# gchochla/VAuLT

Measured on AMD Instinct MI355X. Metric: train samples/sec (img+text pairs) ViLT-B32+BERTweet, bs256, 1/2/4/8 MI355X, higher is better.
Workload: dtype bf16; 1 GPU; ViLT-B32 + bertweet fine-tune step (fwd+bwd+AdamW), per-GPU batch 256, 40 text tokens + 384x384 image (185-token fused sequence; resident as the patch-embedding operand `pixel_patches`, the input pipeline's output), all weights trained; global_batch=256, seq_len=185, parallelism=dp1

## Files before the change

vault_amd/csrc/norm.hip:

```cpp
#include <cstdlib>
#include <algorithm>
#include "common.h"
#include "../../include/vault_hip.h"

namespace {

struct RowMap {
  int rpg, gstride, goff;
  __device__ __forceinline__ size_t operator()(int r) const {
    if (rpg == 0) return (size_t)r;
    const int gq = r / rpg;
    return (size_t)gq * gstride + goff + (r - gq * rpg);
  }
};

template <int VPT>
__global__ __launch_bounds__(256) void ln_fwd_kernel(const float* __restrict__ x, RowMap xmap,
                                                     const float* __restrict__ gamma,
                                                     const float* __restrict__ beta, float eps, int rows, int H,
                                                     h16* __restrict__ y_bf16, float* __restrict__ y_f32, RowMap ymap,
                                                     const float* __restrict__ post_add,
                                                     float* __restrict__ mean, float* __restrict__ rstd,
                                                     uint32_t drop_thresh, uint32_t drop_seed, uint32_t drop_stream,
                                                     float drop_scale, h16* __restrict__ y_split3,
                                                     uint8_t* __restrict__ y_q, uint8_t* __restrict__ y_scale) {
  H16_SATURATE();
  const int lane = threadIdx.x & 63;
  const int row = blockIdx.x * 4 + (threadIdx.x >> 6);
  if (row >= rows) return;
  const float* xr = x + xmap(row) * H;
  f32x4 v[VPT];
  float s = 0.f;
#pragma unroll
  for (int j = 0; j < VPT; ++j) {
    v[j] = *reinterpret_cast<const f32x4*>(xr + (lane + 64 * j) * 4);
    s += v[j][0] + v[j][1] + v[j][2] + v[j][3];
  }
  const float mu = wave_sum(s) / (float)H;
  float q = 0.f;
#pragma unroll
  for (int j = 0; j < VPT; ++j)
#pragma unroll
    for (int e = 0; e < 4; ++e) {
      const float d = v[j][e] - mu;
      q += d * d;
    }
  const float var = wave_sum(q) / (float)H;
  const float rs = 1.0f / sqrtf(var + eps);
  if (lane == 0) {
    if (mean) mean[row] = mu;
    if (rstd) rstd[row] = rs;
  }
  const size_t orow = ymap(row);
#pragma unroll
  for (int j = 0; j < VPT; ++j) {
    const int c = (lane + 64 * j) * 4;
    const f32x4 gw = *reinterpret_cast<const f32x4*>(gamma + c);
    const f32x4 bw = *reinterpret_cast<const f32x4*>(beta + c);
    f32x4 o;
#pragma unroll
    for (int e = 0; e < 4; ++e) o[e] = (v[j][e] - mu) * rs * gw[e] + bw[e];
    if (drop_thresh != 0u) {
#pragma unroll
      for (int e = 0; e < 4; ++e)
        o[e] = dropout_keep(drop_seed, drop_stream, (uint32_t)(orow * H + c + e), drop_thresh) ? o[e] * drop_scale : 0.f;
    }
    if (post_add) {
      const f32x4 pa = *reinterpret_cast<const f32x4*>(post_add + c);
#pragma unroll
      for (int e = 0; e < 4; ++e) o[e] += pa[e];
    }
    if (y_f32) *reinterpret_cast<f32x4*>(y_f32 + orow * H + c) = o;
    if (y_bf16) {
      uint2 w = {pack_h16x2(o[0], o[1]), pack_h16x2(o[2], o[3])};
      *reinterpret_cast<uint2*>(y_bf16 + orow * H + c) = w;
    }
    if (y_q) {
      float b[4];
      float amax = 0.f;
#pragma unroll
      for (int e = 0; e < 4; ++e) { b[e] = (float)(h16)o[e]; amax = fmaxf(amax, fabsf(b[e])); }
      amax = fmaxf(amax, __shfl_xor(amax, 1, 64));
      amax = fmaxf(amax, __shfl_xor(amax, 2, 64));
      amax = fmaxf(amax, __shfl_xor(amax, 4, 64));
      int e8 = 0;
      if (amax > 0.f) {
        e8 = (int)((__builtin_bit_cast(uint32_t, amax) >> 23) & 0xff) - 8;
        e8 = e8 < 0 ? 0 : e8;
      }
      const float inv = __builtin_bit_cast(float, (uint32_t)(254 - e8) << 23);
#pragma unroll
      for (int e = 0; e < 4; ++e) b[e] = fminf(fmaxf(b[e] * inv, -448.f), 448.f);
      int w8 = 0;
      w8 = __builtin_amdgcn_cvt_pk_fp8_f32(b[0], b[1], w8, false);
      w8 = __builtin_amdgcn_cvt_pk_fp8_f32(b[2], b[3], w8, true);
      *reinterpret_cast<int*>(y_q + orow * H + c) = w8;
      if ((lane & 7) == 0) y_scale[orow * (H / 32) + (c >> 5)] = (uint8_t)e8;
    }
    if (y_split3) {
      h16 hi[4], lo[4];
#pragma unroll
      for (int e = 0; e < 4; ++e) split_bf16(o[e], hi[e], lo[e]);
      const uint2 wh = {pack_h16x2((float)hi[0], (float)hi[1]), pack_h16x2((float)hi[2], (float)hi[3])};
      const uint2 wl = {pack_h16x2((float)lo[0], (float)lo[1]), pack_h16x2((float)lo[2], (float)lo[3])};
      h16* d = y_split3 + orow * 3 * H + c;
      *reinterpret_cast<uint2*>(d) = wh;
      *reinterpret_cast<uint2*>(d + H) = wl;
      *reinterpret_cast<uint2*>(d + 2 * H) = wh;
    }
  }
}

template <int VPT, int WAVES>
__device__ __forceinline__ void ln_bwd_fold(const f32x4 (&ag)[VPT], const f32x4 (&ab)[VPT], const f32x4 (&ac)[VPT], float* red,
                                            float* dgamma, float* dbeta, float* dbias, int lane, int wave) {
  constexpr int NB = WAVES >= 8 ? 8 : 4;
  constexpr int HH = VPT * 256;
  if (dgamma == nullptr && dbias == nullptr) return;
  float* const dsts[3] = {dgamma, dbeta, dbias};
  for (int r = 0; r < WAVES / NB; ++r) {
    if ((wave / NB) == r) {
      float* rw = red + (wave % NB) * (3 * HH);
#pragma unroll
      for (int qn = 0; qn < 3; ++qn) {
        if (dsts[qn] == nullptr) continue;
#pragma unroll
        for (int j = 0; j < VPT; ++j) {
          const f32x4 v = qn == 0 ? ag[j] : (qn == 1 ? ab[j] : ac[j]);
          f32x4* q4 = reinterpret_cast<f32x4*>(rw + qn * HH + (lane + 64 * j) * 4);
          *q4 = (r == 0) ? v : (*q4 + v);
        }
      }
    }
    __syncthreads();
  }
  for (int c = threadIdx.x; c < 3 * HH; c += WAVES * 64) {
    const int qn = c / HH;
    float* dst = dsts[qn];
    if (dst == nullptr) continue;
    float t = 0.f;
#pragma unroll
    for (int b = 0; b < NB; ++b) t += red[b * (3 * HH) + c];
    atomicAdd(dst + (c - qn * HH), t);
  }
}

template <int VPT, int WAVES>
__global__ __launch_bounds__(WAVES * 64, 16 / WAVES) void ln_bwd_kernel(const h16* __restrict__ dy_bf16, const float* __restrict__ dy_f32,
                                                     RowMap dymap, const float* __restrict__ x, RowMap xmap,
                                                     const float* __restrict__ mean, const float* __restrict__ rstd,
                                                     const float* __restrict__ gamma, int rows, int H,
                                                     const float* __restrict__ dres, float* __restrict__ dx_f32,
                                                     h16* __restrict__ dx_bf16, RowMap dxmap, float* __restrict__ dgamma,
                                                     float* __restrict__ dbeta, float* __restrict__ dbias,
                                                     int rows_per_block, uint32_t drop_thresh, uint32_t drop_seed, uint32_t drop_stream,
                                                     float drop_scale, int drop_on_dy, const h16* __restrict__ dres_bf16) {
  H16_SATURATE();
  constexpr int NB = WAVES >= 8 ? 8 : 4;
  constexpr int HH = VPT * 256;
  extern __shared__ __attribute__((aligned(16))) float red[];
  const int lane = threadIdx.x & 63, wave = threadIdx.x >> 6;
  f32x4 gw[VPT], ag[VPT], ab[VPT], ac[VPT];
#pragma unroll
  for (int j = 0; j < VPT; ++j) {
    gw[j] = *reinterpret_cast<const f32x4*>(gamma + (lane + 64 * j) * 4);
    ag[j] = f32x4{0.f, 0.f, 0.f, 0.f};
    ab[j] = f32x4{0.f, 0.f, 0.f, 0.f};
    ac[j] = f32x4{0.f, 0.f, 0.f, 0.f};
  }
  const int r0 = blockIdx.x * rows_per_block;
  const int r1 = min(rows, r0 + rows_per_block);
  for (int row = r0 + wave; row < r1; row += WAVES) {
    const size_t xr = xmap(row) * H, dr = dymap(row) * H;
    const float mu = mean[row], rs = rstd[row];
    f32x4 xh[VPT], gy[VPT];
    float s1 = 0.f, s2 = 0.f;
#pragma unroll
    for (int j = 0; j < VPT; ++j) {
      const int c = (lane + 64 * j) * 4;
      const f32x4 xv = *reinterpret_cast<const f32x4*>(x + xr + c);
      f32x4 d = f32x4{0.f, 0.f, 0.f, 0.f};
      if (dy_f32) d = *reinterpret_cast<const f32x4*>(dy_f32 + dr + c);
      if (dy_bf16) {
        const uint2 w = *reinterpret_cast<const uint2*>(dy_bf16 + dr + c);
        const float2 a = unpack_h16x2(w.x), b = unpack_h16x2(w.y);
        d[0] += a.x; d[1] += a.y; d[2] += b.x; d[3] += b.y;
      }
      if (drop_on_dy && drop_thresh != 0u) {
#pragma unroll
        for (int e = 0; e < 4; ++e)
          d[e] = dropout_keep(drop_seed, drop_stream, (uint32_t)(dr + c + e), drop_thresh) ? d[e] * drop_scale : 0.f;
      }
#pragma unroll
      for (int e = 0; e < 4; ++e) {
        xh[j][e] = (xv[e] - mu) * rs;
        gy[j][e] = d[e] * gw[j][e];
        s1 += gy[j][e];
        s2 += gy[j][e] * xh[j][e];
        ag[j][e] += d[e] * xh[j][e];
        ab[j][e] += d[e];
      }
    }
    s1 = wave_sum(s1) / (float)H;
    s2 = wave_sum(s2) / (float)H;
    const size_t orow = dxmap(row) * H;
#pragma unroll
    for (int j = 0; j < VPT; ++j) {
      const int c = (lane + 64 * j) * 4;
      f32x4 o;
#pragma unroll
      for (int e = 0; e < 4; ++e) o[e] = rs * (gy[j][e] - s1 - xh[j][e] * s2);
      if (dres) {
        const f32x4 rv = *reinterpret_cast<const f32x4*>(dres + orow + c);
#pragma unroll
        for (int e = 0; e < 4; ++e) o[e] += rv[e];
      }
      if (dres_bf16) {
        const uint2 w = *reinterpret_cast<const uint2*>(dres_bf16 + orow + c);
        const float2 a = unpack_h16x2(w.x), b = unpack_h16x2(w.y);
        o[0] += a.x; o[1] += a.y; o[2] += b.x; o[3] += b.y;
      }
      if (dx_f32) *reinterpret_cast<f32x4*>(dx_f32 + orow + c) = o;
      if (dx_bf16) {
        if (drop_thresh != 0u && !drop_on_dy) {
#pragma unroll
          for (int e = 0; e < 4; ++e)
            o[e] = dropout_keep(drop_seed, drop_stream, (uint32_t)(orow + c + e), drop_thresh) ? o[e] * drop_scale : 0.f;
        }
        uint2 w = {pack_h16x2(o[0], o[1]), pack_h16x2(o[2], o[3])};
        *reinterpret_cast<uint2*>(dx_bf16 + orow + c) = w;
#pragma unroll
        for (int e = 0; e < 4; ++e) ac[j][e] += o[e];
      }
    }
  }
  ln_bwd_fold<VPT, WAVES>(ag, ab, ac, red, dgamma, dbeta, dbias, lane, wave);
}

template <int VPT>
__global__ __launch_bounds__(512, 1) void ln_bwd_stream_kernel(const h16* __restrict__ dy, const float* __restrict__ x,
                                                                const float* __restrict__ mean, const float* __restrict__ rstd,
                                                                const float* __restrict__ gamma, int rows, int H,
                                                                const h16* __restrict__ dres, h16* __restrict__ dx,
                                                                float* __restrict__ dgamma, float* __restrict__ dbeta,
                                                                float* __restrict__ dbias, int rows_per_block) {
  H16_SATURATE();
  constexpr int WAVES = 8;
  extern __shared__ __attribute__((aligned(16))) float red[];
  const int lane = threadIdx.x & 63, wave = threadIdx.x >> 6;
  f32x4 gw[VPT], ag[VPT], ab[VPT], ac[VPT];
#pragma unroll
  for (int j = 0; j < VPT; ++j) {
    gw[j] = *reinterpret_cast<const f32x4*>(gamma + (lane + 64 * j) * 4);
    ag[j] = f32x4{0.f, 0.f, 0.f, 0.f};
    ab[j] = f32x4{0.f, 0.f, 0.f, 0.f};
    ac[j] = f32x4{0.f, 0.f, 0.f, 0.f};
  }
  const int r0 = blockIdx.x * rows_per_block;
  const int r1 = min(rows, r0 + rows_per_block);
  struct RowRegs {
    f32x4 x[VPT];
    uint2 d[VPT], r[VPT];
    float mu, rs;
  };
  auto request = [&](RowRegs& q, int row) {
    const size_t o = (size_t)row * H;
#pragma unroll
    for (int j = 0; j < VPT; ++j) {
      const int c = (lane + 64 * j) * 4;
      q.x[j] = *reinterpret_cast<const f32x4*>(x + o + c);
      q.d[j] = *reinterpret_cast<const uint2*>(dy + o + c);
      q.r[j] = *reinterpret_cast<const uint2*>(dres + o + c);
    }
    q.mu = mean[row]; q.rs = rstd[row];
  };
  auto process = [&](const RowRegs& q, int row) {
    const float mu = q.mu, rs = q.rs;
    float s1 = 0.f, s2 = 0.f;
#pragma unroll
    for (int j = 0; j < VPT; ++j) {
      const float2 a = unpack_h16x2(q.d[j].x), b = unpack_h16x2(q.d[j].y);
      const float d[4] = {a.x, a.y, b.x, b.y};
#pragma unroll
      for (int e = 0; e < 4; ++e) {
        const float xh = (q.x[j][e] - mu) * rs;
        const float gy = d[e] * gw[j][e];
        s1 += gy;
        s2 += gy * xh;
        ag[j][e] += d[e] * xh;
        ab[j][e] += d[e];
      }
    }
    s1 = wave_sum(s1) / (float)H;
    s2 = wave_sum(s2) / (float)H;
    const size_t o = (size_t)row * H;
#pragma unroll
    for (int j = 0; j < VPT; ++j) {
      const int c = (lane + 64 * j) * 4;
      const float2 a = unpack_h16x2(q.d[j].x), b = unpack_h16x2(q.d[j].y);
      const float2 ra = unpack_h16x2(q.r[j].x), rb = unpack_h16x2(q.r[j].y);
      const float d[4] = {a.x, a.y, b.x, b.y};
      const float r[4] = {ra.x, ra.y, rb.x, rb.y};
      float out[4];
#pragma unroll
      for (int e = 0; e < 4; ++e) {
        const float xh = (q.x[j][e] - mu) * rs;
        out[e] = rs * (d[e] * gw[j][e] - s1 - xh * s2) + r[e];
        ac[j][e] += out[e];
      }
      uint2 w = {pack_h16x2(out[0], out[1]), pack_h16x2(out[2], out[3])};
      *reinterpret_cast<uint2*>(dx + o + c) = w;
    }
  };
  RowRegs qa, qb, qc;
  int row = r0 + wave;
  if (row < r1) request(qa, row);
  if (row + WAVES < r1) request(qb, row + WAVES);
  for (; row < r1; row += 3 * WAVES) {
    if (row + 2 * WAVES < r1) request(qc, row + 2 * WAVES);
    process(qa, row);
    if (row + WAVES >= r1) break;
    if (row + 3 * WAVES < r1) request(qa, row + 3 * WAVES);
    process(qb, row + WAVES);
    if (row + 2 * WAVES >= r1) break;
    if (row + 4 * WAVES < r1) request(qb, row + 4 * WAVES);
    process(qc, row + 2 * WAVES);
  }
  ln_bwd_fold<VPT, WAVES>(ag, ab, ac, red, dgamma, dbeta, dbias, lane, wave);
}

__global__ __launch_bounds__(1024) void colsum_kernel(const h16* __restrict__ in, int ld, int rows, int rows_per_block,
                                                      float* __restrict__ out, long long batch_in, long long batch_out) {
  __shared__ float red[16][256];
  in += (size_t)blockIdx.z * batch_in;
  out += (size_t)blockIdx.z * batch_out;
  const int lane = threadIdx.x & 63, wave = threadIdx.x >> 6;
  const int c0 = blockIdx.x * 256 + lane * 4;
  const int r0 = blockIdx.y * rows_per_block;
  const int r1 = min(rows, r0 + rows_per_block);
  float a0 = 0.f, a1 = 0.f, a2 = 0.f, a3 = 0.f;
  for (int r = r0 + wave; r < r1; r += 16) {
    const uint2 w = *reinterpret_cast<const uint2*>(in + (size_t)r * ld + c0);
    const float2 x = unpack_h16x2(w.x), y = unpack_h16x2(w.y);
    a0 += x.x; a1 += x.y; a2 += y.x; a3 += y.y;
  }
  red[wave][lane * 4] = a0; red[wave][lane * 4 + 1] = a1; red[wave][lane * 4 + 2] = a2; red[wave][lane * 4 + 3] = a3;
  __syncthreads();
  if (threadIdx.x < 256) {
    const int c = threadIdx.x;
    float t = 0.f;
#pragma unroll
    for (int w = 0; w < 16; ++w) t += red[w][c];
    atomicAdd(out + blockIdx.x * 256 + c, t);
  }
}

__global__ __launch_bounds__(1024) void colsum_hm_kernel(const h16* __restrict__ in, int rows, int hm_rows, int rows_per_block,
                                                         float* __restrict__ out, long long batch_in, long long batch_out) {
  __shared__ float red[128][65];
  const h16* base = in + (size_t)blockIdx.z * batch_in + (size_t)blockIdx.x * hm_rows * 64;
  const int t = threadIdx.x, r_in = t >> 3, c8 = (t & 7) * 8;
  const int r0 = blockIdx.y * rows_per_block, r1 = min(rows, r0 + rows_per_block);
  float a[8] = {0.f, 0.f, 0.f, 0.f, 0.f, 0.f, 0.f, 0.f};
  auto add = [&](const u32x4& w) {
#pragma unroll
    for (int k = 0; k < 4; ++k) {
      const float2 x = unpack_h16x2(w[k]);
      a[2 * k] += x.x; a[2 * k + 1] += x.y;
    }
  };
  int r = r0 + r_in;
  for (; r + 128 < r1; r += 256) {
    const u32x4 w0 = *reinterpret_cast<const u32x4*>(base + (size_t)r * 64 + c8);
    const u32x4 w1 = *reinterpret_cast<const u32x4*>(base + (size_t)(r + 128) * 64 + c8);
    add(w0); add(w1);
  }
  if (r < r1) add(*reinterpret_cast<const u32x4*>(base + (size_t)r * 64 + c8));
#pragma unroll
  for (int k = 0; k < 8; ++k) red[r_in][c8 + k] = a[k];
  __syncthreads();
  if (t < 64) {
    float s_ = 0.f;
#pragma unroll 8
    for (int q = 0; q < 128; ++q) s_ += red[q][t];
    atomicAdd(out + (size_t)blockIdx.z * batch_out + blockIdx.x * 64 + t, s_);
  }
}

}

extern "C" int vault_layernorm_fwd(const vault_ln_fwd_args* a, void* stream) {
  if (!a || a->H % 256 || (a->H > 1024 && a->H != 1536) || a->rows <= 0) return VAULT_EINVAL;
  hipStream_t st = reinterpret_cast<hipStream_t>(stream);
  const RowMap xm{a->x_rpg, a->x_gstride, a->x_goff}, ym{a->y_rpg, a->y_gstride, a->y_goff};
  dim3 grid((a->rows + 3) / 4), block(256);
#define LN_FWD(V)                                                                                          \
  hipLaunchKernelGGL(ln_fwd_kernel<V>, grid, block, 0, st, a->x, xm, a->gamma, a->beta, a->eps, a->rows,   \
                     a->H, reinterpret_cast<h16*>(a->y_bf16), a->y_f32, ym, a->post_add, a->mean, a->rstd, \
                     a->drop_thresh, a->drop_seed, a->drop_stream, a->drop_scale, reinterpret_cast<h16*>(a->y_split3), \
                     reinterpret_cast<uint8_t*>(a->y_q), reinterpret_cast<uint8_t*>(a->y_scale))
  switch (a->H / 256) {
    case 1: LN_FWD(1); break;
    case 2: LN_FWD(2); break;
    case 3: LN_FWD(3); break;
    case 4: LN_FWD(4); break;
    case 6: LN_FWD(6); break;
  }
#undef LN_FWD
  return (int)hipGetLastError();
}

extern "C" int vault_layernorm_bwd(const vault_ln_bwd_args* a, void* stream) {
  if (!a || a->H % 256 || (a->H > 1024 && a->H != 1536) || a->rows <= 0) return VAULT_EINVAL;
  hipStream_t st = reinterpret_cast<hipStream_t>(stream);
  const RowMap dym{a->dy_rpg, a->dy_gstride, a->dy_goff}, xm{a->x_rpg, a->x_gstride, a->x_goff},
      dxm{a->dx_rpg, a->dx_gstride, a->dx_goff};
  constexpr int waves = 16;
  const int maxb = 4096 / waves;
  int rpb = (a->rows + maxb - 1) / maxb;
  rpb = ((rpb + waves - 1) / waves) * waves;
  dim3 grid((a->rows + rpb - 1) / rpb), block(waves * 64);
  int lds_bytes = 0;
  const bool ident = a->dy_rpg == 0 && a->x_rpg == 0 && a->dx_rpg == 0;
  if (a->H == 768 && ident && a->dy_bf16 && !a->dy_f32 && !a->dres && a->dres_bf16 && !a->dx_f32 &&
      a->dx_bf16 && a->drop_thresh == 0 && a->dgamma && a->dbeta) {
    constexpr int LDS = 8 * 3 * 768 * 4;
    static bool done[64] = {};
    int dev = 0;
    if (hipGetDevice(&dev) != hipSuccess || dev < 0 || dev >= 64) return VAULT_EINVAL;
    if (!done[dev]) {
      if (hipFuncSetAttribute(reinterpret_cast<const void*>(&ln_bwd_stream_kernel<3>), hipFuncAttributeMaxDynamicSharedMemorySize,
                              LDS) != hipSuccess) return VAULT_EINVAL;
      done[dev] = true;
    }
    int rpb8 = (a->rows + 255) / 256;
    rpb8 = ((rpb8 + 7) / 8) * 8;
    hipLaunchKernelGGL((ln_bwd_stream_kernel<3>), dim3((a->rows + rpb8 - 1) / rpb8), dim3(512), LDS, st,
                       reinterpret_cast<const h16*>(a->dy_bf16), a->x, a->mean,
                       a->rstd, a->gamma, a->rows, a->H, reinterpret_cast<const h16*>(a->dres_bf16),
                       reinterpret_cast<h16*>(a->dx_bf16), a->dgamma, a->dbeta, a->dbias, rpb8);
    return (int)hipGetLastError();
  }
#define LN_BWD(V) LN_BWD_W(V, 16)
#define LN_BWD_W(V, W)                                                                                              \
  {                                                                                                                 \
  {                                                                                                                 \
    constexpr int LDS = (W >= 8 ? 8 : 4) * 3 * V * 256 * 4;                                                         \
    if (LDS > 64 * 1024) {                                                                                          \
      static bool done[64] = {};                                                                                    \
      int dev = 0;                                                                                                  \
      if (hipGetDevice(&dev) != hipSuccess || dev < 0 || dev >= 64) return VAULT_EINVAL;                            \
      if (!done[dev]) {                                                                                             \
        if (hipFuncSetAttribute(reinterpret_cast<const void*>(&ln_bwd_kernel<V, W>),                                \
                                hipFuncAttributeMaxDynamicSharedMemorySize, LDS) != hipSuccess) return VAULT_EINVAL; \
        done[dev] = true;                                                                                           \
      }                                                                                                             \
    }                                                                                                               \
    lds_bytes = LDS;                                                                                                \
  }                                                                                                                 \
  hipLaunchKernelGGL((ln_bwd_kernel<V, W>), grid, block, lds_bytes, st, reinterpret_cast<const h16*>(a->dy_bf16), a->dy_f32, \
                     dym, a->x, xm, a->mean, a->rstd, a->gamma, a->rows, a->H, a->dres, a->dx_f32,               \
                     reinterpret_cast<h16*>(a->dx_bf16), dxm, a->dgamma, a->dbeta, a->dbias, rpb, a->drop_thresh,          \
                     a->drop_seed, a->drop_stream, a->drop_scale, a->drop_on_dy, reinterpret_cast<const h16*>(a->dres_bf16)); \
  }
  switch (a->H / 256) {
    case 1: LN_BWD(1); break;
    case 2: LN_BWD(2); break;
    case 3: LN_BWD(3); break;
    case 4: LN_BWD(4); break;
    case 6: LN_BWD(6); break;
  }
#undef LN_BWD
#undef LN_BWD_W
  return (int)hipGetLastError();
}

__global__ __launch_bounds__(256) void colsum_partials_kernel(const float* __restrict__ part, int nparts, int n,
                                                              float* __restrict__ out, long long batch_in, long long batch_out) {
  const int c = blockIdx.x * 256 + threadIdx.x;
  if (c >= n) return;
  const int per = (nparts + (int)gridDim.z - 1) / (int)gridDim.z;
  const int r0 = blockIdx.z * per, r1 = min(nparts, r0 + per);
  const float* p = part + (size_t)blockIdx.y * batch_in + c;
  float a0 = 0.f, a1 = 0.f, a2 = 0.f, a3 = 0.f;
  int r = r0;
  for (; r + 3 < r1; r += 4) {
    a0 += p[(size_t)r * n]; a1 += p[(size_t)(r + 1) * n]; a2 += p[(size_t)(r + 2) * n]; a3 += p[(size_t)(r + 3) * n];
  }
  for (; r < r1; ++r) a0 += p[(size_t)r * n];
  if (r1 > r0) atomicAdd(out + (size_t)blockIdx.y * batch_out + c, (a0 + a1) + (a2 + a3));
}

extern "C" int vault_colsum_partials(const float* part, int nparts, int n, float* out, int batch, long long batch_in,
                                     long long batch_out, void* stream) {
  if (!part || !out || nparts <= 0 || n <= 0 || batch <= 0 || batch > 65535) return VAULT_EINVAL;
  const int slices = nparts >= 64 ? 16 : 1;
  hipLaunchKernelGGL(colsum_partials_kernel, dim3((n + 255) / 256, batch, slices), dim3(256), 0,
                     reinterpret_cast<hipStream_t>(stream), part, nparts, n, out, batch_in, batch_out);
  return (int)hipGetLastError();
}

extern "C" int vault_colsum_hm(const void* in_bf16, int rows, int hm_rows, int planes, float* out, int batch, long long batch_in,
                               long long batch_out, void* stream) {
  if (!in_bf16 || !out || rows <= 0 || hm_rows < rows || planes <= 0 || batch <= 0 || batch > 65535 || (batch_in & 3))
    return VAULT_EINVAL;
  const int row_blocks = std::max(4, 256 / (planes * batch));
  int rpb = (rows + row_blocks - 1) / row_blocks;
  rpb = ((rpb + 127) / 128) * 128;
  dim3 grid(planes, (rows + rpb - 1) / rpb, batch);
  hipLaunchKernelGGL(colsum_hm_kernel, grid, dim3(1024), 0, reinterpret_cast<hipStream_t>(stream),
                     reinterpret_cast<const h16*>(in_bf16), rows, hm_rows, rpb, out, batch_in, batch_out);
  return (int)hipGetLastError();
}

extern "C" int vault_colsum(const void* in_bf16, int ld, int rows, int N, float* out, void* stream) {
  if (!in_bf16 || !out || N % 256 || rows <= 0) return VAULT_EINVAL;
  const int row_blocks = 256;
  int rpb = (rows + row_blocks - 1) / row_blocks;
  rpb = ((rpb + 15) / 16) * 16;
  dim3 grid(N / 256, (rows + rpb - 1) / rpb);
  hipLaunchKernelGGL(colsum_kernel, grid, dim3(1024), 0, reinterpret_cast<hipStream_t>(stream),
                     reinterpret_cast<const h16*>(in_bf16), ld, rows, rpb, out, 0ll, 0ll);
  return (int)hipGetLastError();
}

extern "C" int vault_colsum_batched(const void* in_bf16, int ld, int rows, int N, float* out, int batch, long long batch_in,
                                    long long batch_out, void* stream) {
  if (!in_bf16 || !out || N % 256 || rows <= 0 || batch <= 0 || batch > 65535 || (batch_in & 3)) return VAULT_EINVAL;
  const int row_blocks = std::max(16, 256 / batch);
  int rpb = (rows + row_blocks - 1) / row_blocks;
  rpb = ((rpb + 15) / 16) * 16;
  dim3 grid(N / 256, (rows + rpb - 1) / rpb, batch);
  hipLaunchKernelGGL(colsum_kernel, grid, dim3(1024), 0, reinterpret_cast<hipStream_t>(stream),
                     reinterpret_cast<const h16*>(in_bf16), ld, rows, rpb, out, batch_in, batch_out);
  return (int)hipGetLastError();
}
```

vault_amd/csrc/optim.hip:

```cpp
#include "common.h"
#include "../../include/vault_hip.h"

namespace {

__global__ __launch_bounds__(256) void adamw_kernel(float* __restrict__ p, float* __restrict__ g, float* __restrict__ m,
                                                    float* __restrict__ v, h16* __restrict__ pb, long long n4,
                                                    float step_size, float lr_wd, float b1, float b2, float eps,
                                                    float gscale, int zero_grad, const uint8_t* __restrict__ zmask) {
  H16_SATURATE();
  for (long long i = blockIdx.x * 256ll + threadIdx.x; i < n4; i += (long long)gridDim.x * 256ll) {
    f32x4 pv = reinterpret_cast<f32x4*>(p)[i];
    f32x4 gv = reinterpret_cast<f32x4*>(g)[i];
    f32x4 mv = reinterpret_cast<f32x4*>(m)[i];
    f32x4 vv = reinterpret_cast<f32x4*>(v)[i];
    if (lr_wd == 0.f) {
      bool idle = true;
#pragma unroll
      for (int e = 0; e < 4; ++e) idle = idle && gv[e] == 0.f && mv[e] == 0.f && vv[e] == 0.f;
      if (idle) continue;
    }
#pragma unroll
    for (int e = 0; e < 4; ++e) {
      const float ge = gv[e] * gscale;
      mv[e] = mv[e] * b1 + (1.f - b1) * ge;
      vv[e] = vv[e] * b2 + (1.f - b2) * ge * ge;
      pv[e] = pv[e] - step_size * (mv[e] / (sqrtf(vv[e]) + eps));
      if (lr_wd != 0.f) pv[e] = pv[e] - lr_wd * pv[e];
    }
    reinterpret_cast<f32x4*>(p)[i] = pv;
    reinterpret_cast<f32x4*>(m)[i] = mv;
    reinterpret_cast<f32x4*>(v)[i] = vv;
    if (zero_grad && (zmask == nullptr || zmask[i >> 4])) reinterpret_cast<f32x4*>(g)[i] = f32x4{0.f, 0.f, 0.f, 0.f};
    if (pb) {
      uint2 w = {pack_h16x2(pv[0], pv[1]), pack_h16x2(pv[2], pv[3])};
      reinterpret_cast<uint2*>(pb)[i] = w;
    }
  }
}

__global__ __launch_bounds__(256) void cast_bf16_kernel(const float* __restrict__ x, h16* __restrict__ y, long long n4) {
  H16_SATURATE();
  for (long long i = blockIdx.x * 256ll + threadIdx.x; i < n4; i += (long long)gridDim.x * 256ll) {
    const f32x4 a = reinterpret_cast<const f32x4*>(x)[i];
    uint2 w = {pack_h16x2(a[0], a[1]), pack_h16x2(a[2], a[3])};
    reinterpret_cast<uint2*>(y)[i] = w;
  }
}

__global__ __launch_bounds__(256) void h16_census_kernel(const uint16_t* __restrict__ x, long long n,
                                                         unsigned long long* __restrict__ out) {
#ifdef VAULT_F16
  constexpr uint16_t EXP = 0x7C00, MAN = 0x03FF, MAXF = 0x7BFF;
#else
  constexpr uint16_t EXP = 0x7F80, MAN = 0x007F, MAXF = 0x7F7F;
#endif
  unsigned c[4] = {0u, 0u, 0u, 0u};
  for (long long i = blockIdx.x * 256ll + threadIdx.x; i < n; i += (long long)gridDim.x * 256ll) {
    const uint16_t a = x[i] & 0x7FFF;
    c[0] += a == MAXF;
    c[1] += (a & EXP) == EXP;
    c[2] += (a & EXP) == 0 && (a & MAN) != 0;
    c[3] += a == 0;
  }
#pragma unroll
  for (int k = 0; k < 4; ++k) {
    unsigned v = c[k];
#pragma unroll
    for (int o = 32; o > 0; o >>= 1) v += __shfl_xor(v, o, 64);
    if ((threadIdx.x & 63) == 0 && v) atomicAdd(out + k, (unsigned long long)v);
  }
}

__global__ __launch_bounds__(256) void split3_kernel(const float* __restrict__ x, h16* __restrict__ out, long long rows,
                                                     int K, int layout) {
  H16_SATURATE();
  const long long total = rows * (long long)(K / 4);
  for (long long i = blockIdx.x * 256ll + threadIdx.x; i < total; i += (long long)gridDim.x * 256ll) {
    const long long r = i / (K / 4);
    const int c = (int)(i - r * (K / 4)) * 4;
    const f32x4 a = *reinterpret_cast<const f32x4*>(x + r * K + c);
    h16 hi[4], lo[4];
#pragma unroll
    for (int e = 0; e < 4; ++e) split_bf16(a[e], hi[e], lo[e]);
    h16* o = out + r * 3 * K + c;
    const uint2 wh = {pack_h16x2((float)hi[0], (float)hi[1]), pack_h16x2((float)hi[2], (float)hi[3])};
    const uint2 wl = {pack_h16x2((float)lo[0], (float)lo[1]), pack_h16x2((float)lo[2], (float)lo[3])};
    *reinterpret_cast<uint2*>(o) = wh;
    *reinterpret_cast<uint2*>(o + K) = layout == 0 ? wl : wh;
    *reinterpret_cast<uint2*>(o + 2 * K) = layout == 0 ? wh : wl;
  }
}

}

extern "C" int vault_split3_bf16(const float* x, void* out_bf16, long long rows, int K, int layout, void* stream) {
  if (!x || !out_bf16 || rows <= 0 || K <= 0 || (K & 3)) return VAULT_EINVAL;
  const long long total = rows * (K / 4);
  const int blocks = (int)((total + 255) / 256 > 8192 ? 8192 : (total + 255) / 256);
  hipLaunchKernelGGL(split3_kernel, dim3(blocks), dim3(256), 0, reinterpret_cast<hipStream_t>(stream), x,
                     reinterpret_cast<h16*>(out_bf16), rows, K, layout);
  return (int)hipGetLastError();
}

extern "C" int vault_adamw_step(float* p, float* g, float* m, float* v, void* p_bf16, long long n, float lr,
                                float beta1, float beta2, float eps, float weight_decay, float bias_corr_factor,
                                float grad_scale, int zero_grad, const unsigned char* zero_mask, void* stream) {
  if (!p || !g || !m || !v || n <= 0 || (n & 3) || (zero_mask && (n & 63))) return VAULT_EINVAL;
  const long long n4 = n / 4;
  const int blocks = (int)((n4 + 255) / 256 > 8192 ? 8192 : (n4 + 255) / 256);
  hipLaunchKernelGGL(adamw_kernel, dim3(blocks), dim3(256), 0, reinterpret_cast<hipStream_t>(stream), p, g, m, v,
                     reinterpret_cast<h16*>(p_bf16), n4, lr * bias_corr_factor, lr * weight_decay, beta1, beta2, eps,
                     grad_scale, zero_grad, zero_mask);
  return (int)hipGetLastError();
}

extern "C" int vault_h16_census(const void* x_h16, long long n, unsigned long long* out4, void* stream) {
  if (!x_h16 || !out4 || n <= 0) return VAULT_EINVAL;
  const int blocks = (int)((n + 255) / 256 > 4096 ? 4096 : (n + 255) / 256);
  hipLaunchKernelGGL(h16_census_kernel, dim3(blocks), dim3(256), 0, reinterpret_cast<hipStream_t>(stream),
                     reinterpret_cast<const uint16_t*>(x_h16), n, out4);
  return (int)hipGetLastError();
}

extern "C" int vault_cast_bf16(const float* x, void* y_bf16, long long n, void* stream) {
  if (!x || !y_bf16 || n <= 0 || (n & 3)) return VAULT_EINVAL;
  const long long n4 = n / 4;
  const int blocks = (int)((n4 + 255) / 256 > 8192 ? 8192 : (n4 + 255) / 256);
  hipLaunchKernelGGL(cast_bf16_kernel, dim3(blocks), dim3(256), 0, reinterpret_cast<hipStream_t>(stream), x,
                     reinterpret_cast<h16*>(y_bf16), n4);
  return (int)hipGetLastError();
}

__global__ __launch_bounds__(256) void transpose_bf16_kernel(const h16* __restrict__ src, h16* __restrict__ dst, int rows,
                                                             int cols, long long stride_src, long long stride_dst) {
  __shared__ h16 tile[64][72];
  const int tiles_c = cols >> 6;
  const int tr = blockIdx.x / tiles_c, tc = blockIdx.x - tr * tiles_c;
  const h16* s = src + (size_t)blockIdx.y * stride_src + (size_t)(tr * 64) * cols + tc * 64;
  h16* d = dst + (size_t)blockIdx.y * stride_dst + (size_t)(tc * 64) * rows + tr * 64;
  const int t = threadIdx.x;
#pragma unroll
  for (int k = 0; k < 2; ++k) {
    const int r = (t >> 3) + 32 * k, c8 = (t & 7) * 8;
    const h16x8 v = *reinterpret_cast<const h16x8*>(s + (size_t)r * cols + c8);
#pragma unroll
    for (int e = 0; e < 8; ++e) tile[r][c8 + e] = v[e];
  }
  __syncthreads();
#pragma unroll
  for (int k = 0; k < 2; ++k) {
    const int c = (t >> 3) + 32 * k, r8 = (t & 7) * 8;
    h16x8 v;
#pragma unroll
    for (int e = 0; e < 8; ++e) v[e] = tile[r8 + e][c];
    *reinterpret_cast<h16x8*>(d + (size_t)c * rows + r8) = v;
  }
}

extern "C" int vault_transpose_bf16(const void* src, void* dst, int rows, int cols, int batch, long long stride_src,
                                    long long stride_dst, void* stream) {
  if (!src || !dst || rows <= 0 || cols <= 0 || (rows & 63) || (cols & 63) || batch <= 0 || batch > 65535 ||
      (stride_src & 7) || (stride_dst & 7))
    return VAULT_EINVAL;
  hipLaunchKernelGGL(transpose_bf16_kernel, dim3((rows >> 6) * (cols >> 6), batch), dim3(256), 0,
                     reinterpret_cast<hipStream_t>(stream), reinterpret_cast<const h16*>(src),
                     reinterpret_cast<h16*>(dst), rows, cols, stride_src, stride_dst);
  return (int)hipGetLastError();
}
```

vault_amd/csrc/optim_clip.hip:

```cpp
#include <math.h>

#include "common.h"
#include "../../include/vault_hip.h"

namespace {

constexpr int NORM_BLOCKS = VAULT_GRAD_NORM_PARTIALS;

__device__ __forceinline__ double sq4(f32x4 a, double acc) {
#pragma unroll
  for (int e = 0; e < 4; ++e) acc = fma((double)a[e], (double)a[e], acc);
  return acc;
}

__device__ __forceinline__ double block_sum(double x, double* ws) {
#pragma unroll
  for (int o = 32; o > 0; o >>= 1) x += __shfl_xor(x, o, 64);
  if ((threadIdx.x & 63) == 0) ws[threadIdx.x >> 6] = x;
  __syncthreads();
  return (ws[0] + ws[1]) + (ws[2] + ws[3]);
}

__global__ __launch_bounds__(256) void sqnorm_partials_kernel(const float* __restrict__ g, long long n4,
                                                              double* __restrict__ partials) {
  __shared__ double ws[4];
  const f32x4* G = reinterpret_cast<const f32x4*>(g);
  const long long stride = (long long)gridDim.x * 256ll;
  long long i = blockIdx.x * 256ll + threadIdx.x;
  double acc = 0.0;
  for (; i + 3 * stride < n4; i += 4 * stride) {
    const f32x4 a = G[i], b = G[i + stride], c = G[i + 2 * stride], d = G[i + 3 * stride];
    acc = sq4(d, sq4(c, sq4(b, sq4(a, acc))));
  }
  for (; i < n4; i += stride) acc = sq4(G[i], acc);
  const double s = block_sum(acc, ws);
  if (threadIdx.x == 0) partials[blockIdx.x] = s;
}

__global__ __launch_bounds__(256) void norm_finish_kernel(const double* __restrict__ partials, int nparts,
                                                          float* __restrict__ out, float max_norm, float unscale) {
  __shared__ double ws[4];
  double acc = 0.0;
  for (int k = threadIdx.x; k < nparts; k += 256) acc += partials[k];
  const double s = block_sum(acc, ws);
  if (threadIdx.x == 0) {
    const float norm = (float)(sqrt(s) * fabs((double)unscale));
    const float c = (1.f / (norm + 1e-6f)) * max_norm;
    out[0] = norm;
    out[1] = c > 1.f ? 1.f : c;
  }
}

__global__ __launch_bounds__(256) void adamw_grouped_kernel(float* __restrict__ p, float* __restrict__ g, float* __restrict__ m,
                                                            float* __restrict__ v, h16* __restrict__ pb, long long n4,
                                                            const uint8_t* __restrict__ gmap, const float* __restrict__ table,
                                                            int n_groups, float lr_factor, float bias_corr, float b1, float b2,
                                                            float eps, float gscale, const float* __restrict__ coef,
                                                            int zero_grad, const uint8_t* __restrict__ zmask) {
  H16_SATURATE();
  __shared__ float2 tab[256];
  {
    const int t = threadIdx.x;
    float2 e = {__builtin_nanf(""), __builtin_nanf("")};
    if (t < n_groups) {
      const float lr = lr_factor * table[2 * t];
      e = {lr * bias_corr, lr * table[2 * t + 1]};
    }
    tab[t] = e;
  }
  const float gs = coef ? gscale * coef[0] : gscale;
  __syncthreads();
  for (long long i = blockIdx.x * 256ll + threadIdx.x; i < n4; i += (long long)gridDim.x * 256ll) {
    const float2 sw = tab[gmap[i >> 4]];
    const float step_size = sw.x, lr_wd = sw.y;
    f32x4 pv = reinterpret_cast<f32x4*>(p)[i];
    f32x4 gv = reinterpret_cast<f32x4*>(g)[i];
    f32x4 mv = reinterpret_cast<f32x4*>(m)[i];
    f32x4 vv = reinterpret_cast<f32x4*>(v)[i];
    if (lr_wd == 0.f) {
      bool idle = true;
#pragma unroll
      for (int e = 0; e < 4; ++e) idle = idle && gv[e] == 0.f && mv[e] == 0.f && vv[e] == 0.f;
      if (idle) continue;
    }
#pragma unroll
    for (int e = 0; e < 4; ++e) {
      const float ge = gv[e] * gs;
      mv[e] = mv[e] * b1 + (1.f - b1) * ge;
      vv[e] = vv[e] * b2 + (1.f - b2) * ge * ge;
      pv[e] = pv[e] - step_size * (mv[e] / (sqrtf(vv[e]) + eps));
      if (lr_wd != 0.f) pv[e] = pv[e] - lr_wd * pv[e];
    }
    reinterpret_cast<f32x4*>(p)[i] = pv;
    reinterpret_cast<f32x4*>(m)[i] = mv;
    reinterpret_cast<f32x4*>(v)[i] = vv;
    if (zero_grad && (zmask == nullptr || zmask[i >> 4])) reinterpret_cast<f32x4*>(g)[i] = f32x4{0.f, 0.f, 0.f, 0.f};
    if (pb) {
      uint2 w = {pack_h16x2(pv[0], pv[1]), pack_h16x2(pv[2], pv[3])};
      reinterpret_cast<uint2*>(pb)[i] = w;
    }
  }
}

}

extern "C" int vault_grad_norm(const float* g, long long n, double* partials, float* out2, float max_norm, float unscale,
                               void* stream) {
  if (!g || !partials || !out2 || n <= 0 || (n & 3) || !(max_norm > 0.f)) return VAULT_EINVAL;
  const long long n4 = n / 4;
  const int blocks = (int)((n4 + 255) / 256 > NORM_BLOCKS ? NORM_BLOCKS : (n4 + 255) / 256);
  hipStream_t s = reinterpret_cast<hipStream_t>(stream);
  hipLaunchKernelGGL(sqnorm_partials_kernel, dim3(blocks), dim3(256), 0, s, g, n4, partials);
  hipLaunchKernelGGL(norm_finish_kernel, dim3(1), dim3(256), 0, s, partials, blocks, out2, max_norm, unscale);
  return (int)hipGetLastError();
}

extern "C" int vault_adamw_step_grouped(float* p, float* g, float* m, float* v, void* p_bf16, long long n,
                                        const unsigned char* group_map, const float* group_table, int n_groups,
                                        float lr_factor, float beta1, float beta2, float eps, float bias_corr_factor,
                                        float grad_scale, const float* coef, int zero_grad, const unsigned char* zero_mask,
                                        void* stream) {
  if (!p || !g || !m || !v || !group_map || !group_table || n <= 0 || (n & 3) || (zero_mask && (n & 63)) ||
      n_groups < 1 || n_groups > 256)
    return VAULT_EINVAL;
  const long long n4 = n / 4;
  const int blocks = (int)((n4 + 255) / 256 > 8192 ? 8192 : (n4 + 255) / 256);
  hipLaunchKernelGGL(adamw_grouped_kernel, dim3(blocks), dim3(256), 0, reinterpret_cast<hipStream_t>(stream), p, g, m, v,
                     reinterpret_cast<h16*>(p_bf16), n4, group_map, group_table, n_groups, lr_factor, bias_corr_factor,
                     beta1, beta2, eps, grad_scale, coef, zero_grad, zero_mask);
  return (int)hipGetLastError();
}
```

Measured before the change: 6776 samples/s.

## Restructure AdamW into prefetched unrolled streaming loop with nontemporal access

```diff
diff --git a/vault_amd/csrc/adamw_loop.h b/vault_amd/csrc/adamw_loop.h
--- /dev/null
+++ b/vault_amd/csrc/adamw_loop.h
@@ -0,0 +1,159 @@
+#pragma once
+#include "common.h"
+
+#ifndef ADAMW_U
+#define ADAMW_U 4
+#endif
+#ifndef ADAMW_NT
+#define ADAMW_NT 1
+#endif
+#ifndef ADAMW_PF
+#define ADAMW_PF 1
+#endif
+
+namespace adamw {
+
+typedef __attribute__((ext_vector_type(2))) uint32_t u32x2;
+constexpr int U = ADAMW_U;
+constexpr int CHUNK = 64 * U;
+constexpr int THREADS = 256;
+constexpr int WAVES = THREADS / 64;
+
+template <typename T>
+__device__ __forceinline__ T ld(const T* p) {
+#if ADAMW_NT
+  return __builtin_nontemporal_load(p);
+#else
+  return *p;
+#endif
+}
+template <typename T>
+__device__ __forceinline__ void st(T* p, T v) {
+#if ADAMW_NT
+  __builtin_nontemporal_store(v, p);
+#else
+  *p = v;
+#endif
+}
+
+struct OneGroup {
+  float step_size, lr_wd;
+  __device__ __forceinline__ uint32_t fetch(long long) const { return 0u; }
+  __device__ __forceinline__ float2 get(uint32_t) const { return float2{step_size, lr_wd}; }
+};
+struct GroupMap {
+  const uint8_t* gmap;
+  const float2* tab;
+  __device__ __forceinline__ uint32_t fetch(long long i) const { return gmap[i >> 4]; }
+  __device__ __forceinline__ float2 get(uint32_t k) const { return tab[k]; }
+};
+
+struct Regs {
+  f32x4 p[U], g[U], m[U], v[U];
+  uint32_t zm[U], grp[U];
+};
+
+template <class G>
+__device__ __forceinline__ void run(float* __restrict__ p, float* __restrict__ g, float* __restrict__ m,
+                                    float* __restrict__ v, h16* __restrict__ pb, long long n4, float b1, float b2,
+                                    float eps, float gscale, int zero_grad, const uint8_t* __restrict__ zmask,
+                                    const G& grp) {
+  f32x4* const P = reinterpret_cast<f32x4*>(p);
+  f32x4* const Gr = reinterpret_cast<f32x4*>(g);
+  f32x4* const M = reinterpret_cast<f32x4*>(m);
+  f32x4* const V = reinterpret_cast<f32x4*>(v);
+  const int lane = threadIdx.x & 63;
+  const int wave = __builtin_amdgcn_readfirstlane((int)(threadIdx.x >> 6));
+  const long long nchunks = (n4 + CHUNK - 1) / CHUNK;
+  const long long stride = (long long)gridDim.x * WAVES;
+
+  auto request = [&](Regs& q, long long c) {
+    const long long i0 = c * CHUNK + lane;
+#pragma unroll
+    for (int u = 0; u < U; ++u) {
+      const long long i = i0 + 64 * u < n4 ? i0 + 64 * u : n4 - 1;
+      q.p[u] = ld(P + i);
+      q.g[u] = ld(Gr + i);
+      q.m[u] = ld(M + i);
+      q.v[u] = ld(V + i);
+      q.zm[u] = *(zmask ? zmask + (i >> 4) : reinterpret_cast<const uint8_t*>(P + i));
+      q.grp[u] = grp.fetch(i);
+    }
+  };
+  auto process = [&](Regs& q, long long c) {
+    const long long i0 = c * CHUNK + lane;
+#pragma unroll
+    for (int u = 0; u < U; ++u) {
+      const long long i = i0 + 64 * u;
+      if (i >= n4) continue;
+      const float2 sw = grp.get(q.grp[u]);
+      const float step_size = sw.x, lr_wd = sw.y;
+      f32x4 pv = q.p[u], mv = q.m[u], vv = q.v[u];
+      const f32x4 gv = q.g[u];
+      if (lr_wd == 0.f) {
+        bool idle = true;
+#pragma unroll
+        for (int e = 0; e < 4; ++e) idle = idle && gv[e] == 0.f && mv[e] == 0.f && vv[e] == 0.f;
+        if (idle) continue;
+      }
+#pragma unroll
+      for (int e = 0; e < 4; ++e) {
+        const float ge = gv[e] * gscale;
+        mv[e] = mv[e] * b1 + (1.f - b1) * ge;
+        vv[e] = vv[e] * b2 + (1.f - b2) * ge * ge;
+        pv[e] = pv[e] - step_size * (mv[e] / (sqrtf(vv[e]) + eps));
+        if (lr_wd != 0.f) pv[e] = pv[e] - lr_wd * pv[e];
+      }
+      st(P + i, pv);
+      st(M + i, mv);
+      st(V + i, vv);
+      if (zero_grad && (zmask == nullptr || q.zm[u])) st(Gr + i, f32x4{0.f, 0.f, 0.f, 0.f});
+      if (pb) {
+        const u32x2 w = {pack_h16x2(pv[0], pv[1]), pack_h16x2(pv[2], pv[3])};
+        st(reinterpret_cast<u32x2*>(pb) + i, w);
+      }
+    }
+  };
+
+  long long c = blockIdx.x * (long long)WAVES + wave;
+  if (c >= nchunks) return;
+#if ADAMW_PF
+  Regs qa, qb;
+  request(qa, c);
+  for (;;) {
+    if (c + stride >= nchunks) { process(qa, c); break; }
+    request(qb, c + stride);
+    process(qa, c);
+    c += stride;
+    if (c + stride >= nchunks) { process(qb, c); break; }
+    request(qa, c + stride);
+    process(qb, c);
+    c += stride;
+  }
+#else
+  Regs qa;
+  for (; c < nchunks; c += stride) {
+    request(qa, c);
+    process(qa, c);
+  }
+#endif
+}
+
+template <class K>
+inline int grid_blocks(K kernel, long long n4, int* blocks) {
+  static int resident[64] = {};
+  int dev = 0;
+  if (hipGetDevice(&dev) != hipSuccess || dev < 0 || dev >= 64) return VAULT_EINVAL;
+  if (!resident[dev]) {
+    int per_cu = 0, cus = 0;
+    if (hipOccupancyMaxActiveBlocksPerMultiprocessor(&per_cu, kernel, THREADS, 0) != hipSuccess || per_cu < 1 ||
+        hipDeviceGetAttribute(&cus, hipDeviceAttributeMultiprocessorCount, dev) != hipSuccess || cus < 1)
+      return VAULT_EINVAL;
+    resident[dev] = per_cu * cus;
+  }
+  const long long want = ((n4 + CHUNK - 1) / CHUNK + WAVES - 1) / WAVES;
+  *blocks = (int)(want < resident[dev] ? want : resident[dev]);
+  return 0;
+}
+
+}
diff --git a/vault_amd/csrc/norm.hip b/vault_amd/csrc/norm.hip
--- a/vault_amd/csrc/norm.hip
+++ b/vault_amd/csrc/norm.hip
@@ -3,7 +3,22 @@
 #include "common.h"
 #include "../../include/vault_hip.h"
 
+#ifndef LN_NT_X
+#define LN_NT_X 1
+#endif
+#ifndef LN_STREAM_ABLATE
+#define LN_STREAM_ABLATE 0
+#endif
+
 namespace {
+
+__device__ __forceinline__ f32x4 ld_x(const float* p) {
+#if LN_NT_X
+  return __builtin_nontemporal_load(reinterpret_cast<const f32x4*>(p));
+#else
+  return *reinterpret_cast<const f32x4*>(p);
+#endif
+}
 
 struct RowMap {
   int rpg, gstride, goff;
@@ -268,9 +283,14 @@
 #pragma unroll
     for (int j = 0; j < VPT; ++j) {
       const int c = (lane + 64 * j) * 4;
-      q.x[j] = *reinterpret_cast<const f32x4*>(x + o + c);
+#if LN_STREAM_ABLATE == 2
+      q.x[j] = f32x4{(float)c, 1.f, (float)row, 2.f};
+      q.d[j] = q.r[j] = uint2{(uint32_t)(o + c), 0x3c003c00u};
+#else
+      q.x[j] = ld_x(x + o + c);
       q.d[j] = *reinterpret_cast<const uint2*>(dy + o + c);
       q.r[j] = *reinterpret_cast<const uint2*>(dres + o + c);
+#endif
     }
     q.mu = mean[row]; q.rs = rstd[row];
   };
@@ -287,8 +307,10 @@
         const float gy = d[e] * gw[j][e];
         s1 += gy;
         s2 += gy * xh;
+#if LN_STREAM_ABLATE != 3
         ag[j][e] += d[e] * xh;
         ab[j][e] += d[e];
+#endif
       }
     }
     s1 = wave_sum(s1) / (float)H;
@@ -306,10 +328,14 @@
       for (int e = 0; e < 4; ++e) {
         const float xh = (q.x[j][e] - mu) * rs;
         out[e] = rs * (d[e] * gw[j][e] - s1 - xh * s2) + r[e];
+#if LN_STREAM_ABLATE != 3
         ac[j][e] += out[e];
-      }
+#endif
+      }
+#if LN_STREAM_ABLATE != 1
       uint2 w = {pack_h16x2(out[0], out[1]), pack_h16x2(out[2], out[3])};
       *reinterpret_cast<uint2*>(dx + o + c) = w;
+#endif
     }
   };
   RowRegs qa, qb, qc;
@@ -326,7 +352,9 @@
     if (row + 4 * WAVES < r1) request(qb, row + 4 * WAVES);
     process(qc, row + 2 * WAVES);
   }
+#if LN_STREAM_ABLATE != 3
   ln_bwd_fold<VPT, WAVES>(ag, ab, ac, red, dgamma, dbeta, dbias, lane, wave);
+#endif
 }
 
 __global__ __launch_bounds__(1024) void colsum_kernel(const h16* __restrict__ in, int ld, int rows, int rows_per_block,
diff --git a/vault_amd/csrc/optim.hip b/vault_amd/csrc/optim.hip
--- a/vault_amd/csrc/optim.hip
+++ b/vault_amd/csrc/optim.hip
@@ -1,41 +1,16 @@
 #include "common.h"
 #include "../../include/vault_hip.h"
+#include "adamw_loop.h"
 
 namespace {
 
-__global__ __launch_bounds__(256) void adamw_kernel(float* __restrict__ p, float* __restrict__ g, float* __restrict__ m,
-                                                    float* __restrict__ v, h16* __restrict__ pb, long long n4,
-                                                    float step_size, float lr_wd, float b1, float b2, float eps,
-                                                    float gscale, int zero_grad, const uint8_t* __restrict__ zmask) {
+__global__ __launch_bounds__(adamw::THREADS) void adamw_kernel(float* __restrict__ p, float* __restrict__ g,
+                                                               float* __restrict__ m, float* __restrict__ v,
+                                                               h16* __restrict__ pb, long long n4, float step_size,
+                                                               float lr_wd, float b1, float b2, float eps, float gscale,
+                                                               int zero_grad, const uint8_t* __restrict__ zmask) {
   H16_SATURATE();
-  for (long long i = blockIdx.x * 256ll + threadIdx.x; i < n4; i += (long long)gridDim.x * 256ll) {
-    f32x4 pv = reinterpret_cast<f32x4*>(p)[i];
-    f32x4 gv = reinterpret_cast<f32x4*>(g)[i];
-    f32x4 mv = reinterpret_cast<f32x4*>(m)[i];
-    f32x4 vv = reinterpret_cast<f32x4*>(v)[i];
-    if (lr_wd == 0.f) {
-      bool idle = true;
-#pragma unroll
-      for (int e = 0; e < 4; ++e) idle = idle && gv[e] == 0.f && mv[e] == 0.f && vv[e] == 0.f;
-      if (idle) continue;
-    }
-#pragma unroll
-    for (int e = 0; e < 4; ++e) {
-      const float ge = gv[e] * gscale;
-      mv[e] = mv[e] * b1 + (1.f - b1) * ge;
-      vv[e] = vv[e] * b2 + (1.f - b2) * ge * ge;
-      pv[e] = pv[e] - step_size * (mv[e] / (sqrtf(vv[e]) + eps));
-      if (lr_wd != 0.f) pv[e] = pv[e] - lr_wd * pv[e];
-    }
-    reinterpret_cast<f32x4*>(p)[i] = pv;
-    reinterpret_cast<f32x4*>(m)[i] = mv;
-    reinterpret_cast<f32x4*>(v)[i] = vv;
-    if (zero_grad && (zmask == nullptr || zmask[i >> 4])) reinterpret_cast<f32x4*>(g)[i] = f32x4{0.f, 0.f, 0.f, 0.f};
-    if (pb) {
-      uint2 w = {pack_h16x2(pv[0], pv[1]), pack_h16x2(pv[2], pv[3])};
-      reinterpret_cast<uint2*>(pb)[i] = w;
-    }
-  }
+  adamw::run(p, g, m, v, pb, n4, b1, b2, eps, gscale, zero_grad, zmask, adamw::OneGroup{step_size, lr_wd});
 }
 
 __global__ __launch_bounds__(256) void cast_bf16_kernel(const float* __restrict__ x, h16* __restrict__ y, long long n4) {
@@ -107,8 +82,9 @@
                                 float grad_scale, int zero_grad, const unsigned char* zero_mask, void* stream) {
   if (!p || !g || !m || !v || n <= 0 || (n & 3) || (zero_mask && (n & 63))) return VAULT_EINVAL;
   const long long n4 = n / 4;
-  const int blocks = (int)((n4 + 255) / 256 > 8192 ? 8192 : (n4 + 255) / 256);
-  hipLaunchKernelGGL(adamw_kernel, dim3(blocks), dim3(256), 0, reinterpret_cast<hipStream_t>(stream), p, g, m, v,
+  int blocks = 0;
+  if (const int rc = adamw::grid_blocks(adamw_kernel, n4, &blocks)) return rc;
+  hipLaunchKernelGGL(adamw_kernel, dim3(blocks), dim3(adamw::THREADS), 0, reinterpret_cast<hipStream_t>(stream), p, g, m, v,
                      reinterpret_cast<h16*>(p_bf16), n4, lr * bias_corr_factor, lr * weight_decay, beta1, beta2, eps,
                      grad_scale, zero_grad, zero_mask);
   return (int)hipGetLastError();
diff --git a/vault_amd/csrc/optim_clip.hip b/vault_amd/csrc/optim_clip.hip
--- a/vault_amd/csrc/optim_clip.hip
+++ b/vault_amd/csrc/optim_clip.hip
@@ -2,6 +2,7 @@
 
 #include "common.h"
 #include "../../include/vault_hip.h"
+#include "adamw_loop.h"
 
 namespace {
 
@@ -51,7 +52,7 @@
   }
 }
 
-__global__ __launch_bounds__(256) void adamw_grouped_kernel(float* __restrict__ p, float* __restrict__ g, float* __restrict__ m,
+__global__ __launch_bounds__(adamw::THREADS) void adamw_grouped_kernel(float* __restrict__ p, float* __restrict__ g, float* __restrict__ m,
                                                             float* __restrict__ v, h16* __restrict__ pb, long long n4,
                                                             const uint8_t* __restrict__ gmap, const float* __restrict__ table,
                                                             int n_groups, float lr_factor, float bias_corr, float b1, float b2,
@@ -70,36 +71,7 @@
   }
   const float gs = coef ? gscale * coef[0] : gscale;
   __syncthreads();
-  for (long long i = blockIdx.x * 256ll + threadIdx.x; i < n4; i += (long long)gridDim.x * 256ll) {
-    const float2 sw = tab[gmap[i >> 4]];
-    const float step_size = sw.x, lr_wd = sw.y;
-    f32x4 pv = reinterpret_cast<f32x4*>(p)[i];
-    f32x4 gv = reinterpret_cast<f32x4*>(g)[i];
-    f32x4 mv = reinterpret_cast<f32x4*>(m)[i];
-    f32x4 vv = reinterpret_cast<f32x4*>(v)[i];
-    if (lr_wd == 0.f) {
-      bool idle = true;
-#pragma unroll
-      for (int e = 0; e < 4; ++e) idle = idle && gv[e] == 0.f && mv[e] == 0.f && vv[e] == 0.f;
-      if (idle) continue;
-    }
-#pragma unroll
-    for (int e = 0; e < 4; ++e) {
-      const float ge = gv[e] * gs;
-      mv[e] = mv[e] * b1 + (1.f - b1) * ge;
-      vv[e] = vv[e] * b2 + (1.f - b2) * ge * ge;
-      pv[e] = pv[e] - step_size * (mv[e] / (sqrtf(vv[e]) + eps));
-      if (lr_wd != 0.f) pv[e] = pv[e] - lr_wd * pv[e];
-    }
-    reinterpret_cast<f32x4*>(p)[i] = pv;
-    reinterpret_cast<f32x4*>(m)[i] = mv;
-    reinterpret_cast<f32x4*>(v)[i] = vv;
-    if (zero_grad && (zmask == nullptr || zmask[i >> 4])) reinterpret_cast<f32x4*>(g)[i] = f32x4{0.f, 0.f, 0.f, 0.f};
-    if (pb) {
-      uint2 w = {pack_h16x2(pv[0], pv[1]), pack_h16x2(pv[2], pv[3])};
-      reinterpret_cast<uint2*>(pb)[i] = w;
-    }
-  }
+  adamw::run(p, g, m, v, pb, n4, b1, b2, eps, gs, zero_grad, zmask, adamw::GroupMap{gmap, tab});
 }
 
 }
@@ -124,8 +96,9 @@
       n_groups < 1 || n_groups > 256)
     return VAULT_EINVAL;
   const long long n4 = n / 4;
-  const int blocks = (int)((n4 + 255) / 256 > 8192 ? 8192 : (n4 + 255) / 256);
-  hipLaunchKernelGGL(adamw_grouped_kernel, dim3(blocks), dim3(256), 0, reinterpret_cast<hipStream_t>(stream), p, g, m, v,
+  int blocks = 0;
+  if (const int rc = adamw::grid_blocks(adamw_grouped_kernel, n4, &blocks)) return rc;
+  hipLaunchKernelGGL(adamw_grouped_kernel, dim3(blocks), dim3(adamw::THREADS), 0, reinterpret_cast<hipStream_t>(stream), p, g, m, v,
                      reinterpret_cast<h16*>(p_bf16), n4, group_map, group_table, n_groups, lr_factor, bias_corr_factor,
                      beta1, beta2, eps, grad_scale, coef, zero_grad, zero_mask);
   return (int)hipGetLastError();
```

Result: no change. 6793 samples/s, median of 5 (+0.3%).
